# ray-project/kuberay

Hardware: NVIDIA H100
Metric: reconciles/sec over 10k RayCluster x 100 pods (batched reconcilePods + status roll-up) (higher is better)
Workload: dtype u32

## Files before the change

### kuberay_b200/csrc/kr_bucket2.cuh

```cuda
#pragma once

#include "kr_decide.cuh"

namespace kr {

__device__ __forceinline__ uint32_t inc_epoch_of(const ScratchDev &sc) { return __ldcg(&sc.inc[KR_INC_EPOCH]) + 1u; }

#ifndef KR_D2WARPS
#define KR_D2WARPS 8
#endif
static constexpr int kD2Warps = KR_D2WARPS;
#define KR_ROW_UNHEALTHY (1u << 13)
#define KR_ROW_FRESH (1u << 14)
#define KR_LG_OWNED (1u << 31)

__device__ __forceinline__ uint4 *large_slot(const ScratchDev &sc, uint32_t c, uint32_t rank) {
  if (!sc.lg) return nullptr;
  const uint4 l = __ldcg(&sc.lg[c]);
  const uint32_t j = rank - sc.bucket_stride;
  return j < l.y ? sc.region + l.x + j : nullptr;
}
__device__ __forceinline__ uint4 *rec_slot(const ScratchDev &sc, uint32_t c, uint32_t rank) {
  return rank < sc.bucket_stride ? sc.bucket + (size_t)c * sc.bucket_stride + rank : large_slot(sc, c, rank);
}
__host__ __device__ __forceinline__ uint32_t large_region_cap(uint32_t count, uint32_t stride) {
  const uint32_t want = ((count + count / 4 + 31) / 32) * 32;
  return (count > KR_LARGE_MAX_PODS ? want : (want < KR_LARGE_MAX_PODS ? want : (uint32_t)KR_LARGE_MAX_PODS)) - stride;
}


template <int kItems>
__global__ void __launch_bounds__(kSortThreads) k_match2(SnapDev s, ScratchDev sc, ResDev r, Sizes n, int has_wtd) {
  KR_TL(1);
  extern __shared__ uint32_t sm_bits[];
  __shared__ uint32_t s_orph[kSortThreads / 32];
  const uint32_t tile = blockIdx.x;
  const uint32_t warp = threadIdx.x >> 5, lane = threadIdx.x & 31;
  const uint32_t base = tile * (kSortThreads * kItems) + warp * (32 * kItems) + lane;
  uint32_t ns[kItems], cn[kItems], gn[kItems], nm[kItems], pk[kItems], ri[kItems];
#pragma unroll
  for (int it = 0; it < kItems; it++) {
    const uint32_t p = base + it * 32;
    const bool v = p < n.n_pods;
    ns[it] = v ? __ldg(&s.p_ns_id[p]) : 0u; cn[it] = v ? __ldg(&s.p_cluster_name_id[p]) : 0u;
    gn[it] = v ? __ldg(&s.p_group_name_id[p]) : 0u; nm[it] = v ? __ldg(&s.p_name_id[p]) : 0u;
    pk[it] = v ? __ldg(&s.p_packed[p]) : 0u; ri[it] = v ? (uint32_t)__ldg(&s.p_replica_index[p]) : 0u;
  }
  pdl_wait(); pdl_trigger();
  uint32_t pi[kItems];
  uint4 sl[kItems];
#pragma unroll
  for (int it = 0; it < kItems; it++) {
    pi[it] = hash_pair(ns[it], cn[it]) & sc.cl_mask;
    sl[it] = __ldg(&sc.cl_slots[pi[it]]);
  }
  if (has_wtd) {
    const uint32_t words = (sc.wt_bits_mask + 1) >> 5;
    for (uint32_t i = threadIdx.x; i < words; i += kSortThreads) sm_bits[i] = __ldcg(&sc.wt_bits[i]);
    __syncthreads();
  }
  uint32_t orphans = 0;
// ... 54 lines not shown
      const int32_t aux = aux_lookup(sc, p);
      const unsigned long long key = ((unsigned long long)p << 32) | (uint32_t)(aux + 1);
      atomicMax(reinterpret_cast<unsigned long long *>(&sc.cl_dyn[c].z), ~key);
    }
    cidx[it] = matched ? c : n.n_clusters;
    roww[it] = (slot << 16) | flags;
    orphans += __popc(__ballot_sync(0xFFFFFFFFu, v && !matched && !(pk[it] & KR_PP_TOMBSTONE)));
  }
  uint32_t rank[kItems];
#pragma unroll
  for (int it = 0; it < kItems; it++) rank[it] = cidx[it] < n.n_clusters ? atomicAdd(&sc.cl_dyn[cidx[it]].x, 1u) : 0u;
#pragma unroll
  for (int it = 0; it < kItems; it++) {
    if (cidx[it] >= n.n_clusters) continue;
    if (rank[it] < sc.bucket_stride) {
      sc.bucket[(size_t)cidx[it] * sc.bucket_stride + rank[it]] = make_uint4(base + it * 32, roww[it], ri[it], nm[it]);
      sc.pos[base + it * 32] = rank[it];
    } else if (uint4 *slot = large_slot(sc, cidx[it], rank[it])) {
      *slot = make_uint4(base + it * 32, roww[it], ri[it], nm[it]);
      sc.pos[base + it * 32] = rank[it];
    } else KR_MARK_ATTEMPT_VOID(r.totals);
  }
  if (lane == 0) s_orph[warp] = orphans;
  __syncthreads();
  if (threadIdx.x == 0) {
    uint32_t t = 0;
#pragma unroll
    for (int w = 0; w < kSortThreads / 32; w++) t += s_orph[w];
    if (t) atomicAdd(&r.totals[1], t);
  }
}


struct IncStage { uint32_t *meta; kr_cluster_result *clusters; kr_group_result *groups; uint32_t cap_clusters, cap_groups; };
// ... 156 lines not shown
    mine = c < a.r.totals[4];
    if (mine) { c = a.sc.deferred_list[c]; in_word = __ldg(&a.sc.cl_in[32 * (size_t)c + lane]); }
  } else if (kInc) {
    mine = c < __ldcg(&a.sc.inc[KR_INC_DIRTY]) && !__ldcg(&a.sc.inc[KR_INC_VOID]) && !__ldcg(&a.sc.inc[KR_INC_STRUCTURAL]);
    if (mine) {
      c = a.sc.dirty_list[c];
      in_word = __ldcg(&a.sc.cl_in[32 * (size_t)c + lane]);
    }
  }
  s_in[warp][lane] = in_word;
  __syncwarp();
  const RecordCI ci{s_in[warp]};
  if (KR_ATTEMPT_VOID(a.r.totals)) mine = false;
  if (ci.group_cnt() > KR_SMEM_GROUPS) mine = false;
  if (kInc && !mine) return;
  uint4 *bucket = a.sc.bucket + (size_t)(mine ? c : 0) * S;
  uint4 dyn = make_uint4(0, 0, 0, 0);
  uint4 recs[K] = {};
  if (mine) {
    dyn = __ldcg(&a.sc.cl_dyn[c]);
#pragma unroll
    for (int k = 0; k < K; k++) if ((uint32_t)(k * 32) + lane < S) recs[k] = __ldcg(&bucket[k * 32 + lane]);
  }
  uint32_t P = dyn.x;
  if (P > S) { mine = false; P = 0; }
  if (kInc) {
    const uint32_t epoch = inc_epoch_of(a.sc);
    const bool lost = dyn.y == epoch;
    uint32_t kept = 0, head_min = 0xFFFFFFFFu;
#pragma unroll
    for (int k = 0; k < K; k++) {
      const uint32_t j = k * 32 + lane;
      bool keep = mine && j < P;
      const bool fresh = keep && (recs[k].y & KR_ROW_FRESH);
      if (keep && lost && !fresh) keep = __ldcg(&a.sc.stamp[recs[k].x]) != epoch;
      const uint32_t bal = __ballot_sync(0xFFFFFFFFu, keep);
      if (keep) {
        uint4 rec = recs[k];
        rec.y &= ~KR_ROW_FRESH;
        const uint32_t to = kept + __popc(bal & lt);
        if (fresh || to != j) { bucket[to] = rec; if (to != j) a.sc.pos[rec.x] = to; }
        if (pp_node_type(rec.y & 0xFFFFu) == KR_NT_HEAD) head_min = min(head_min, rec.x);
      }
      kept += __popc(bal);
    }
    head_min = __reduce_min_sync(0xFFFFFFFFu, head_min);
    __syncwarp();
    unsigned long long raw = 0;
    if (mine) {
      if (lane == 0 && head_min != 0xFFFFFFFFu) raw = ~(((unsigned long long)head_min << 32) | (uint32_t)(aux_lookup(a.sc, head_min) + 1));
      raw = __shfl_sync(0xFFFFFFFFu, raw, 0);
      P = kept;
      dyn = make_uint4(kept, 0u, (uint32_t)raw, (uint32_t)(raw >> 32));
      if (lane == 0) a.sc.cl_dyn[c] = dyn;
    }
#pragma unroll
    for (int k = 0; k < K; k++) recs[k] = mine && (uint32_t)(k * 32) + lane < kept ? __ldcg(&bucket[k * 32 + lane]) : make_uint4(0, 0, 0, 0);
  }
  const uint32_t cf = ci.flags(), G = ci.group_cnt(), g0 = ci.group_off();
  const uint8_t suspend_status = ci.suspend_status(), ext_err = ci.ext_err_kind(), old_prov = ci.cond_status(KR_COND_PROVISIONED);
  const bool gate = a.f.gate_status_conditions != 0;
  if (kInc && mine) {
    uint32_t old_create = 0;
    for (uint32_t gi = lane; gi < G; gi += 32) old_create += a.r.groups[g0 + gi].n_create;
    s_old_create[warp] = __reduce_add_sync(0xFFFFFFFFu, old_create);
  }
  uint32_t head_pod = 0xFFFFFFFFu;
  int32_t head_aux = -1;
  {
    const unsigned long long raw = ((unsigned long long)dyn.w << 32) | dyn.z;
    if (mine && raw != 0) { const unsigned long long key = ~raw; head_pod = (uint32_t)(key >> 32); head_aux = (int32_t)(uint32_t)key - 1; }
  }
// ... 240 lines not shown
          __syncwarp();
#pragma unroll
          for (int k = 0; k < K; k++) {
            const bool isc = ((cand >> k) & 1u) && (pw[k] >> 16) == gi;
            if (!__any_sync(0xFFFFFFFFu, isc)) continue;
            uint32_t rank = 0;
            for (uint32_t i = 0; i < nc; i++) rank += s_list[warp][i] < pidx[k] ? 1u : 0u;
            if (isc && (int32_t)rank < pre) act[k] = KR_ACT_DELETE_RANDOM;
          }
          __syncwarp();
        }
      }
    }
  }
  if (!(cf & KR_CF_SKIP)) {
    const uint32_t head_name = (n_heads == 1 && head_pos != 0xFFFFFFFFu) ? __ldcg(&a.sc.bucket[(size_t)c * S + head_pos].w) : 0u;
    status_rollup(a.s, a.f, ci, cr, P, (uint32_t)n_heads, n_heads > 0 ? (int32_t)head_pod : -1, head_aux, head_name, ready, available, all_running);
  }
  __syncwarp();
  if (mine && lane < sizeof(kr_cluster_result) / 4)
    reinterpret_cast<uint32_t *>(&a.r.clusters[c])[lane] = reinterpret_cast<const volatile uint32_t *>(&cr)[lane];

  uint32_t n_act = 0;
  uint32_t arank[K];
#pragma unroll
  for (int k = 0; k < K; k++) {
    arank[k] = 0;
    const bool isa = act[k] != KR_ACT_KEEP;
    const uint32_t bal = __ballot_sync(0xFFFFFFFFu, isa);
    if (isa) s_list[warp][n_act + __popc(bal & lt)] = pidx[k];
    n_act += __popc(bal);
// ... 76 lines not shown
      if (want == 0) continue;
      if ((uint64_t)off + want > a.create_cap) { off += want; continue; }
      int32_t *out = a.r.create_idx + off;
      if (!a.f.gate_multihost_indexing) {
        for (uint32_t k2 = lane; k2 < want; k2 += 32) out[k2] = -1;
      } else {
        const bool mh = kMH && g_mode[gi] == GM_MULTIHOST;
        const uint64_t bound = (uint64_t)(mh ? g_mh_running[gi] : acc_list[gi] - acc_wtd[gi]) + want;
        uint32_t written = 0;
        for (uint64_t w0 = 0; w0 < bound && written < want; w0 += 1024) {
          s_bits[warp][lane] = 0;
          __syncwarp();
#pragma unroll
          for (int k = 0; k < K; k++) {
            if ((pw[k] >> 16) == gi && (pw[k] & KR_PP_HAS_REPLICA_IDX) && (mh ? ((mh_head >> k) & 1u) != 0 : (act[k] == KR_ACT_KEEP && pidx[k] != 0xFFFFFFFFu))) {
              const int32_t idx = (int32_t)__ldcg(&a.sc.bucket[(size_t)c * S + k * 32 + lane].z);
              if (idx >= 0 && (uint64_t)idx >= w0 && (uint64_t)idx < w0 + 1024 && (uint64_t)idx < bound)
                atomicOr(&s_bits[warp][(idx - w0) >> 5], 1u << ((idx - w0) & 31));
            }
          }
          __syncwarp();
          const uint32_t word = s_bits[warp][lane];
          const uint64_t wbase = w0 + 32ull * lane;
          uint32_t freeb = ~word;
          if (wbase >= bound) freeb = 0;
          else if (bound - wbase < 32) freeb &= (1u << (uint32_t)(bound - wbase)) - 1;
          const uint32_t cnt = __popc(freeb);
          uint32_t x = cnt;
#pragma unroll
          for (int d = 1; d < 32; d <<= 1) { const uint32_t y = __shfl_up_sync(0xFFFFFFFFu, x, d); if (lane >= (uint32_t)d) x += y; }
          uint32_t pos = written + x - cnt;
// ... 22 lines not shown
```

### kuberay_b200/csrc/kr_common.cuh

```cuda
#pragma once

#include <cuda_runtime.h>
#include <stdint.h>

#include "../../include/kr_engine.h"

namespace kr {


struct SnapDev {
  const uint32_t *c_ns_id, *c_name_id;
  const uint64_t *c_uid_hash;
  const uint32_t *c_flags;
  const uint8_t *c_suspend_status, *c_ext_err_kind;
  const uint32_t *c_ext_err_msg_id, *c_group_off, *c_group_cnt;
  const uint64_t *c_json_off;
  const uint32_t *c_json_len;
  const uint8_t *c_old_state;
  const int32_t *c_old_counts;
  const uint8_t *c_old_cond_status, *c_old_cond_variant;
  const uint32_t *c_old_cond_reason_id, *c_old_cond_msg_id, *c_old_head_ids;
  const uint8_t *c_svc_count, *c_svc_ip_kind;
  const uint32_t *c_svc_ip_id, *c_svc_name_id;
  const uint32_t *g_cluster_idx, *g_name_id;
// ... 34 lines not shown
  uint32_t *aux_keys; uint32_t *aux_vals; uint32_t aux_mask;
  uint4 *rows;
  uint32_t *keys[2]; uint32_t *vals[2];
  uint32_t *hist;
  uint32_t *row_total;
  uint32_t *gcreate;
  uint32_t *cact;
  uint32_t *mh_rep, *mh_name, *mh_meta, *mh_cnt, *mh_flg;
  uint8_t *mh_act, *mh_head;
  uint32_t *act_tmp_idx; uint8_t *act_tmp_code;
  uint32_t *tile_orph;
  uint32_t *chain;
  uint32_t *ccount, *cstart;
  uint32_t *deferred_list;
  int32_t *gacc;
  uint4 *bucket; uint32_t bucket_stride;
  uint32_t *wt_bits; uint32_t wt_bits_mask;
  uint32_t *cl_in;
  uint4 *cl_dyn;
  uint32_t *stamp;
  uint32_t *touched;
  uint32_t *touched_old;
  uint32_t *pos;
  uint32_t *dirty_flag;
  uint32_t *obj_flag;
  uint32_t *dirty_list;
  uint32_t *act_res, *cre_res;
  uint32_t *inc;
  uint4 *lg;
  uint4 *region;
};
enum {
  KR_INC_TOUCHED = 0, KR_INC_DIRTY = 1,
  KR_INC_STRUCTURAL = 2,
  KR_INC_EPOCH = 3,
  KR_INC_HEADS = 4,
  KR_INC_VOID = 5,
  KR_INC_GROUPS = 6,
  KR_INC_LSEG = 7,
  KR_INC_GROW = 8,
  KR_INC_SPILL = 9,
  KR_INC_GROWN = 10,
};
enum {
  KR_CI_FLAGS = 0, KR_CI_GOFF = 1, KR_CI_GCNT = 2,
// ... 100 lines not shown
```

### kuberay_b200/csrc/kr_engine.cu

```cuda
#include <cuda_runtime.h>

#include <algorithm>
#include <chrono>
#include <cstdarg>
#include <cstdio>
#include <cstdlib>
#include <cstring>
#include <string>
#include <thread>
#include <unordered_map>
#include <unordered_set>
#include <vector>

#include "kr_kernels.cuh"
#include "kr_incr.cuh"
#include "kr_large.cuh"
#include "kr_huge.cuh"

using namespace kr;

int kr_specjson_emit_string(const uint8_t *spec_json, uint64_t len, bool muted, long max_groups, std::string &out, long *n_groups);

namespace {

// ... 389 lines not shown
  L.cstart = o; o = align_up(o + 4 * ((size_t)n.n_clusters + 2));
  L.tile_orph = o; o = align_up(o + 4 * ((size_t)L.mtiles + 8));
  L.mh_rep = o; o = align_up(o + 4 * (size_t)n.n_pods);
  L.mh_name = o; o = align_up(o + 4 * (size_t)n.n_pods);
  L.mh_meta = o; o = align_up(o + 4 * (size_t)n.n_pods);
  L.mh_cnt = o; o = align_up(o + 4 * (size_t)n.n_pods);
  L.mh_flg = o; o = align_up(o + 4 * (size_t)n.n_pods);
  L.mh_act = o; o = align_up(o + (size_t)n.n_pods);
  L.mh_head = o; o = align_up(o + (size_t)n.n_pods);
  L.act_tmp_idx = o; o = align_up(o + 4 * (size_t)n.n_pods);
  L.act_tmp_code = o; o = align_up(o + (size_t)n.n_pods);
  L.bucket_entries = std::max<size_t>(4 * (size_t)n.n_pods, 64 * (size_t)n.n_clusters);
  L.bucket_entries = std::max<size_t>(L.bucket_entries, std::min<size_t>(256 * (size_t)n.n_clusters, (size_t)4 << 20));
  if (64 * (size_t)n.n_clusters > 8 * (size_t)n.n_pods + (4u << 20)) L.bucket_entries = 0;
  L.cl_in = o; o = align_up(o + 128 * (size_t)n.n_clusters);
  L.bucket = o; o = align_up(o + 16 * L.bucket_entries);
  L.inc_zero = o;
  L.stamp = o; o = align_up(o + 4 * (size_t)n.n_pods);
  L.dirty_flag = o; o = align_up(o + 4 * (size_t)n.n_clusters);
  L.obj_flag = o; o = align_up(o + 4 * (size_t)n.n_clusters);
  L.inc = o; o = align_up(o + 64);
  L.inc_zero_end = o;
  L.touched = o; o = align_up(o + 4 * (size_t)n.n_pods);
  L.touched_old = o; o = align_up(o + 4 * (size_t)n.n_pods);
  L.pos = o; o = align_up(o + 4 * (size_t)n.n_pods);
  L.dirty_list = o; o = align_up(o + 4 * (size_t)n.n_clusters);
  L.act_res = o; o = align_up(o + 4 * (size_t)n.n_clusters);
  L.cre_res = o; o = align_up(o + 4 * (size_t)n.n_clusters);
  L.total = o;
  return L;
}
// ... 64 lines not shown
  bool env_radix = false;
  uint32_t *h_totals = nullptr;
  bool no_bucket = false;
  bool hash_spin = true;
  uint32_t bstride = 0;
  bool large_on = false;
  bool wide_on = false;
  bool huge_on = false;
  std::vector<uint32_t> large_rows; std::vector<uint2> large_reg;
  bool lg_stale = false;
  bool lg_moved = false;
  uint32_t n_large = 0;
  uint32_t n_lsort = 0;
  uint32_t n_tiles = 0;
  uint8_t *d_lg = nullptr;
  uint4 *d_region = nullptr;
  size_t large_entries = 0;
  std::vector<uint4> h_lg; std::vector<uint32_t> h_lg_list;
  uint8_t *d_huge = nullptr;
  size_t huge_tiles = 0;
  std::vector<uint4> h_tiles;
  bool huge_growth = false;
  size_t huge_reserve = 0;
  bool large_growth = false;
  uint4 *d_grow = nullptr; uint4 *h_grow = nullptr;
  size_t lg_cursor = 0;
  bool ran_bucket = false;
  uint64_t h2d_accum = 0;
  uint32_t *h_order = nullptr, *d_order = nullptr;
  cudaEvent_t ev_order = nullptr;
  bool order_pending = false;
// ... 95 lines not shown
  s.vals[0] = reinterpret_cast<uint32_t *>(b + L.vals0); s.vals[1] = reinterpret_cast<uint32_t *>(b + L.vals1);
  s.hist = reinterpret_cast<uint32_t *>(b + L.hist);
  s.row_total = reinterpret_cast<uint32_t *>(b + L.row_total);
  s.gacc = reinterpret_cast<int32_t *>(b + L.gacc);
  s.gcreate = reinterpret_cast<uint32_t *>(b + L.gcreate);
  s.deferred_list = reinterpret_cast<uint32_t *>(b + L.deferred_list);
  s.cact = reinterpret_cast<uint32_t *>(b + L.cact);
  s.ccount = reinterpret_cast<uint32_t *>(b + L.ccount);
  s.chain = reinterpret_cast<uint32_t *>(b + L.chain);
  s.cstart = reinterpret_cast<uint32_t *>(b + L.cstart);
  s.tile_orph = reinterpret_cast<uint32_t *>(b + L.tile_orph);
  s.mh_rep = reinterpret_cast<uint32_t *>(b + L.mh_rep); s.mh_name = reinterpret_cast<uint32_t *>(b + L.mh_name);
  s.mh_meta = reinterpret_cast<uint32_t *>(b + L.mh_meta); s.mh_cnt = reinterpret_cast<uint32_t *>(b + L.mh_cnt);
  s.mh_flg = reinterpret_cast<uint32_t *>(b + L.mh_flg); s.mh_act = b + L.mh_act; s.mh_head = b + L.mh_head;
  s.act_tmp_idx = reinterpret_cast<uint32_t *>(b + L.act_tmp_idx); s.act_tmp_code = b + L.act_tmp_code;
  s.bucket = reinterpret_cast<uint4 *>(b + L.bucket); s.bucket_stride = 0;
  s.wt_bits = reinterpret_cast<uint32_t *>(b + L.wt_bits); s.wt_bits_mask = L.wt_bits_n - 1;
  s.cl_in = reinterpret_cast<uint32_t *>(b + L.cl_in);
  s.cl_dyn = reinterpret_cast<uint4 *>(b + L.cl_dyn);
  s.stamp = reinterpret_cast<uint32_t *>(b + L.stamp); s.touched = reinterpret_cast<uint32_t *>(b + L.touched);
  s.touched_old = reinterpret_cast<uint32_t *>(b + L.touched_old); s.pos = reinterpret_cast<uint32_t *>(b + L.pos);
  s.obj_flag = reinterpret_cast<uint32_t *>(b + L.obj_flag);
  s.dirty_flag = reinterpret_cast<uint32_t *>(b + L.dirty_flag); s.dirty_list = reinterpret_cast<uint32_t *>(b + L.dirty_list);
  s.act_res = reinterpret_cast<uint32_t *>(b + L.act_res); s.cre_res = reinterpret_cast<uint32_t *>(b + L.cre_res);
  s.inc = reinterpret_cast<uint32_t *>(b + L.inc);
  s.lg = nullptr; s.region = nullptr;
  return s;
}

template <typename... KArgs, typename... Args>
cudaError_t launch_pdl(void (*kern)(KArgs...), dim3 grid, dim3 block, size_t smem, cudaStream_t st, bool pdl, Args... args) {
// ... 1033 lines not shown
    e->lg_stale = true;
    return KR_OK;
  }
  if (option == KR_OPT_LARGE_CLUSTERS || option == KR_OPT_WIDE_CLUSTERS || option == KR_OPT_HUGE_CLUSTERS) {
    bool &on = option == KR_OPT_LARGE_CLUSTERS ? e->large_on : option == KR_OPT_WIDE_CLUSTERS ? e->wide_on : e->huge_on;
    if (on == (value != 0)) return KR_OK;
    if (value) CK(cudaSetDevice(e->cfg.device));
    if (value && option != KR_OPT_HUGE_CLUSTERS && !e->d_lg) {
      const size_t Nc = e->cfg.max_clusters;
      CK(cudaMalloc((void **)&e->d_lg, align_up(16 * Nc) + 4 * Nc));
      CK(cudaMemset(e->d_lg, 0, align_up(16 * Nc)));
    }
    if (value && option == KR_OPT_LARGE_CLUSTERS && !e->d_region) {
      const size_t Np = e->cfg.max_pods;
      const size_t entries = Np * 5 / 4 + 32 * (Np / 257 + 1);
      CK(cudaMalloc((void **)&e->d_region, 16 * entries));
      e->large_entries = entries;
    }
    if (value && option == KR_OPT_HUGE_CLUSTERS && !e->d_huge) {
      e->huge_tiles = resident_tiles(e->cfg);
      if (int rc = alloc_huge(e, 0)) return rc;
    }
    on = value != 0;
    if (int rc = drop_regions(e, 0)) return rc;
    e->lg_cursor = 0; e->lg_stale = true; e->inc_valid = false; e->gvalid = false;
    e->force_radix = e->env_radix;
    if (e->begun) e->bstride = first_stride(e->sizes);
    return KR_OK;
  }
  if (option == KR_OPT_BUCKET_STRIDE) return fail(e, KR_E_INVALID, "KR_OPT_BUCKET_STRIDE can only be read");
  return fail(e, KR_E_INVALID, "unknown option %u", option);
// ... 645 lines not shown
```

### kuberay_b200/csrc/kr_huge.cuh

```cuda
#pragma once

#include "kr_large.cuh"

namespace kr {

static constexpr int kHugeThreads = 1024;
static constexpr int kHugePer = kHugeTile / kHugeThreads;

struct HugeDev {
  const uint4 *tiles;
  uint32_t *cnt;
  uint32_t *done;
  uint32_t *runs;
  uint32_t *stash;
};

__device__ __forceinline__ uint32_t gallop_lower_bound(const uint32_t *s, uint32_t lo, uint32_t n, uint32_t x) {
  uint32_t hi = lo, step = 1;
  while (hi < n && s[hi] < x) { lo = hi + 1; hi += step; step <<= 1; }
  hi = min(hi, n);
  while (lo < hi) { const uint32_t mid = (lo + hi) >> 1; if (s[mid] < x) lo = mid + 1; else hi = mid; }
  return lo;
}

// ... 15 lines not shown
    const uint32_t cap = __ldcg(&sc.lg[c].y);
    bool go = !KR_ATTEMPT_VOID(a.r.totals);
    if (kInc) go = go && !__ldcg(&sc.inc[KR_INC_VOID]) && !__ldcg(&sc.inc[KR_INC_STRUCTURAL]) && __ldcg(&sc.dirty_flag[c]) == epoch;
    const bool wide = a.s.c_group_cnt[c] > KR_SMEM_GROUPS;
    s_go = go && (P > S ? P - S <= cap : wide);
    if (!s_go && r0 == 0) sc.lg[c].w = 0;
  }
  __syncthreads();
  if (!s_go) return;
  const bool lost = kInc && dyn.y == epoch;
  const uint32_t r1 = min(P, r0 + (uint32_t)kHugeTile), n = r1 > r0 ? r1 - r0 : 0u;
  const uint32_t per = (n + kHugeThreads - 1) / kHugeThreads;
  const uint32_t j0 = r0 + min(tid * per, n), j1 = min(j0 + per, r1);
  uint32_t kept = 0;
  for (uint32_t j = j0; j < j1; j++) {
    const uint4 rec = __ldcg(rec_slot(sc, c, j));
    const bool keep = !lost || (rec.y & KR_ROW_FRESH) || __ldcg(&sc.stamp[rec.x]) != epoch;
    if (keep) { sc.rows[rec.x] = make_uint4(rec.w, a.s.p_replica_name_id[rec.x], rec.z, rec.y & ~KR_ROW_FRESH); kept++; }
  }
  uint32_t x = kept;
#pragma unroll
  for (int d = 1; d < 32; d <<= 1) { const uint32_t y = __shfl_up_sync(0xFFFFFFFFu, x, d); if (lane >= (uint32_t)d) x += y; }
  if (lane == 31) s_warp[warp] = x;
  __syncthreads();
  uint32_t before = 0, total = 0;
  for (uint32_t w = 0; w < kHugeThreads / 32; w++) { const uint32_t v = s_warp[w]; before += w < warp ? v : 0u; total += v; }
  uint32_t o = before + x - kept;
  uint32_t *stash = h.stash + (size_t)blockIdx.x * kHugeTile;
  for (uint32_t j = j0; j < j1; j++) {
    const uint4 rec = __ldcg(rec_slot(sc, c, j));
    const bool keep = !lost || (rec.y & KR_ROW_FRESH) || __ldcg(&sc.stamp[rec.x]) != epoch;
    if (keep) { s_idx[o] = rec.x; stash[o] = rec.x; o++; }
  }
  block_sort_asc<kHugeThreads>(s_idx, total, tid);
  uint32_t *run = h.runs + (size_t)blockIdx.x * kHugeTile;
  for (uint32_t k = tid; k < total; k += kHugeThreads) run[k] = s_idx[k];
  if (tid == 0) {
    h.cnt[blockIdx.x] = total;
    __threadfence();
    if (atomicAdd(&h.done[t.z], 1u) == t.w - 1) {
      __threadfence();
      uint32_t sum = 0;
      for (uint32_t i = t.z; i < t.z + t.w; i++) sum += __ldcg(&h.cnt[i]);
      const uint32_t seg = atomicAdd(&sc.inc[KR_INC_LSEG], sum);
      sc.lg[c].z = seg; sc.lg[c].w = sum | KR_LG_OWNED;
// ... 34 lines not shown
    const uint32_t *run = h.runs + (size_t)u * kHugeTile;
    for (uint32_t k = tid; k < n_u; k += kHugeThreads) s_run[k] = __ldcg(run + k);
    __syncthreads();
    if (k0 >= n_me) continue;
    uint32_t lo = 0;
#pragma unroll
    for (int i = 0; i < kHugePer; i++) { lo = gallop_lower_bound(s_run, lo, n_u, v[i]); at[i] += lo; }
  }
#pragma unroll
  for (int i = 0; i < kHugePer; i++) if (k0 + i < n_me) a.r.sorted_pod_idx[seg + at[i]] = v[i];
  if (kInc) {
    const uint32_t *stash = h.stash + (size_t)me * kHugeTile;
    for (uint32_t k = tid; k < n_me; k += kHugeThreads) {
      const uint32_t p = __ldcg(stash + k);
      const uint4 row = __ldcg(&sc.rows[p]);
      *rec_slot(sc, c, base + k) = make_uint4(p, row.w, row.z, row.x);
      sc.pos[p] = base + k;
    }
    if (me == t.z && tid == 0) { sc.cl_dyn[c].x = total; sc.cl_dyn[c].y = 0u; }
  }
}

}
```

### kuberay_b200/csrc/kr_incr.cuh

```cuda
#pragma once

#include "kr_bucket2.cuh"

namespace kr {

__device__ __forceinline__ uint32_t inc_epoch(const ScratchDev &sc) { return inc_epoch_of(sc); }

__device__ __forceinline__ void mark_dirty(const ScratchDev &sc, uint32_t c, uint32_t epoch) {
  if (atomicExch(&sc.dirty_flag[c], epoch) != epoch) sc.dirty_list[atomicAdd(&sc.inc[KR_INC_DIRTY], 1u)] = c;
}

__device__ __forceinline__ bool cl_probe(const ScratchDev &sc, uint32_t ns, uint32_t name, uint32_t &c, uint32_t &cflags, uint32_t &gname0) {
  if (name == 0) return false;
  uint32_t i = hash_pair(ns, name) & sc.cl_mask;
  while (true) {
    const uint4 q = __ldcg(&sc.cl_slots[i]);
    if (q.x == name && q.y == ns) { c = q.w >> 2; cflags = q.w & 3u; gname0 = q.z; return true; }
    if (q.x == KR_EMPTY32 && q.y == KR_EMPTY32) return false;
    i = (i + 1) & sc.cl_mask;
  }
}

__device__ __forceinline__ bool inc_touch(const SnapDev &s, const ScratchDev &sc, const ResDev &r, uint32_t p, uint32_t epoch, uint32_t n_resident, uint32_t &ns, uint32_t &nm) {
  if (atomicExch(&sc.stamp[p], epoch) == epoch) return false;
// ... 213 lines not shown

__global__ void __launch_bounds__(256) k_inc_refresh(SnapDev s, ScratchDev sc) {
  const uint32_t n_dirty = __ldcg(&sc.inc[KR_INC_DIRTY]);
  const uint32_t epoch = inc_epoch(sc);
  if (__ldcg(&sc.inc[KR_INC_STRUCTURAL])) return;
  for (uint32_t i = blockIdx.x * blockDim.x + threadIdx.x; i < n_dirty; i += gridDim.x * blockDim.x) {
    const uint32_t c = sc.dirty_list[i];
    if (__ldcg(&sc.obj_flag[c]) == epoch) write_cl_in(s, sc, c, s.c_group_off[c], s.c_group_cnt[c]);
  }
}

static constexpr uint32_t kGrowResult = KR_GROW_MAX, kGrowSpill = 2 * KR_GROW_MAX;
static constexpr size_t kGrowBytes = 16 * ((size_t)kGrowSpill + 2 * (size_t)KR_GROW_SPILL);

__device__ __noinline__ bool grow_spill(const uint4 *lg, uint32_t *inc, uint32_t *pos, uint32_t stride, uint4 *grow, uint32_t c,
                                        uint32_t rank, uint4 rec) {
  const uint4 l = __ldcg(&lg[c]);
  if (rank == stride + l.y) {
    const uint32_t j = atomicAdd(&inc[KR_INC_GROW], 1u);
    if (j >= KR_GROW_MAX) return false;
    grow[j] = make_uint4(c, l.x, l.y, 0u);
  }
  const uint32_t k = atomicAdd(&inc[KR_INC_SPILL], 1u);
  if (k >= KR_GROW_SPILL) return false;
  grow[kGrowSpill + 2 * k] = make_uint4(rec.x, rank, c, 0u);
  grow[kGrowSpill + 2 * k + 1] = rec;
  pos[rec.x] = rank;
  return true;
}

__global__ void __launch_bounds__(256) k_inc_admit(SnapDev s, ScratchDev sc, ResDev r, Sizes n, int has_wtd, uint4 *grow) {
  const uint32_t n_touched = __ldcg(&sc.inc[KR_INC_TOUCHED]);
  const uint32_t epoch = inc_epoch(sc);
  if (__ldcg(&sc.inc[KR_INC_STRUCTURAL])) return;
  for (uint32_t i = blockIdx.x * blockDim.x + threadIdx.x; i < n_touched; i += gridDim.x * blockDim.x) {
    const uint32_t p = sc.touched[i], c_old = sc.touched_old[i];
    if (p >= n.n_pods) continue;
    const uint32_t ns = s.p_ns_id[p], cn = s.p_cluster_name_id[p], gn = s.p_group_name_id[p], nm = s.p_name_id[p], pk = s.p_packed[p];
    const uint32_t ri = (uint32_t)s.p_replica_index[p];
    uint32_t c = n.n_clusters, cflags = 0, gname0 = 0;
    const bool matched = cl_probe(sc, ns, cn, c, cflags, gname0);
    uint32_t slot = KR_ROW_NO_GROUP, g0 = 0xFFFFFFFFu;
    if (matched && gn != 0) {
      if (gname0 == gn) slot = 0;
      else if (cflags & KR_CL_MULTI) {
        const uint4 rec = sc.cl_rec[c];
        g0 = rec.x;
        for (uint32_t gi = 1; gi < rec.y; gi++)
          if (s.g_name_id[g0 + gi] == gn) { slot = gi; break; }
      }
    }
    uint32_t flags = pk & (0x7FFu | KR_PP_TOMBSTONE);
    if (should_delete(pk)) flags |= KR_ROW_UNHEALTHY;
    if (has_wtd) {
// ... 8 lines not shown
              atomicMin(&r.wtd_pod_idx[e], p);
              if (slot != KR_ROW_NO_GROUP) {
                if (g0 == 0xFFFFFFFFu) g0 = s.c_group_off[c];
                const uint32_t g = g0 + slot, off = s.g_wtd_off[g];
                if (e >= off && e < off + s.g_wtd_cnt[g]) flags |= KR_ROW_WTD_OWN;
              }
            }
            break;
          }
          j = (j + 1) & sc.wt_mask;
          kk = __ldcg(&sc.wt_keys[j]);
        }
      }
    }
    if (matched && c == c_old) {
      uint4 *at = rec_slot(sc, c, sc.pos[p]);
      if (!at) { sc.inc[KR_INC_VOID] = 1u; continue; }
      *at = make_uint4(p, (slot << 16) | flags, ri, nm);
      sc.stamp[p] = 0u;
      continue;
    }
    if (c_old != KR_EMPTY32) sc.cl_dyn[c_old].y = epoch;
    if (!matched) {
      if (!(pk & KR_PP_TOMBSTONE)) atomicAdd(&r.totals[1], 1u);
      continue;
    }
    mark_dirty(sc, c, epoch);
    const uint32_t rank = atomicAdd(&sc.cl_dyn[c].x, 1u);
    const uint4 rec = make_uint4(p, (slot << 16) | flags | KR_ROW_FRESH, ri, nm);
    if (uint4 *at = rec_slot(sc, c, rank)) { *at = rec; sc.pos[p] = rank; }
    else if (!grow || !grow_spill(sc.lg, sc.inc, sc.pos, sc.bucket_stride, grow, c, rank, rec)) sc.inc[KR_INC_VOID] = 1u;
  }
}

__global__ void __launch_bounds__(256) k_inc_clusters_insert(SnapDev s, ScratchDev sc, ResDev r, const uint32_t *rows, uint32_t n, int names) {
  const uint32_t i = blockIdx.x * blockDim.x + threadIdx.x;
  if (i >= n || __ldcg(&sc.inc[KR_INC_STRUCTURAL])) return;
  const uint32_t c = rows[i];
  cl_insert_cluster(s, sc, c);
  sc.cl_dyn[c] = make_uint4(0u, 0u, 0u, 0u);
  sc.act_res[c] = 0u; sc.cre_res[c] = 0u;
  r.act_start[c] = 0u; r.act_cnt[c] = 0u;
  if (sc.lg) sc.lg[c] = make_uint4(0u, 0u, 0u, 0u);
  const uint32_t g0 = s.c_group_off[c], G = s.c_group_cnt[c];
  for (uint32_t g = g0; g < g0 + G; g++) {
// ... 44 lines not shown

__global__ void __launch_bounds__(256) k_inc_digest_move(const uint32_t *__restrict__ pairs, uint32_t n, char *hash) {
  const uint32_t t = blockIdx.x * blockDim.x + threadIdx.x;
  if (t >= 2 * n) return;
  const uint32_t from = pairs[2 * (t >> 1)], to = pairs[2 * (t >> 1) + 1];
  reinterpret_cast<uint4 *>(hash + 32 * (size_t)to)[t & 1] = reinterpret_cast<const uint4 *>(hash + 32 * (size_t)from)[t & 1];
}

__global__ void __launch_bounds__(256) k_inc_clusters_release(SnapDev s, ScratchDev sc, ResDev r, const uint32_t *gone, uint32_t n_gone, uint32_t n_resident) {
  const uint32_t w = (blockIdx.x * blockDim.x + threadIdx.x) >> 5, lane = threadIdx.x & 31;
  if (w >= n_gone) return;
  const uint32_t o = gone[w], epoch = inc_epoch(sc);
  const uint4 rec = sc.cl_rec[o];
  const uint32_t P = sc.cl_dyn[o].x;
  for (uint32_t k = lane; k < P; k += 32) {
    const uint4 *at = rec_slot(sc, o, k);
    uint32_t ns, nm;
    if (at) inc_touch(s, sc, r, at->x, epoch, n_resident, ns, nm);
  }
  uint32_t cre = 0;
  for (uint32_t g = rec.x + lane; g < rec.x + rec.y; g += 32) cre += r.groups[g].n_create;
  cre = __reduce_add_sync(0xFFFFFFFFu, cre);
  if (lane == 0) {
    if (r.act_cnt[o]) atomicSub(&r.totals[2], r.act_cnt[o]);
    if (cre) atomicSub(&r.totals[6], cre);
  }
}

__global__ void __launch_bounds__(256) k_inc_large_release(SnapDev s, ScratchDev sc, ResDev r, const uint4 *gone, uint32_t n_resident) {
  __shared__ uint32_t s_cre[8];
  const uint4 g = gone[blockIdx.x];
  const uint32_t o = g.x, S = sc.bucket_stride, epoch = inc_epoch(sc), tid = threadIdx.x;
  const uint32_t P = min(__ldcg(&sc.cl_dyn[o].x), S + g.z);
  for (uint32_t k = tid; k < P; k += blockDim.x) {
    const uint4 *at = k < S ? sc.bucket + (size_t)o * S + k : sc.region + g.y + (k - S);
    uint32_t ns, nm;
    inc_touch(s, sc, r, at->x, epoch, n_resident, ns, nm);
  }
  const uint4 rec = sc.cl_rec[o];
  uint32_t cre = 0;
  for (uint32_t gi = rec.x + tid; gi < rec.x + rec.y; gi += blockDim.x) cre += r.groups[gi].n_create;
  cre = __reduce_add_sync(0xFFFFFFFFu, cre);
  if ((tid & 31) == 0) s_cre[tid >> 5] = cre;
  __syncthreads();
  if (tid == 0) {
    cre = 0;
    for (uint32_t w = 0; w < blockDim.x / 32; w++) cre += s_cre[w];
    if (r.act_cnt[o]) atomicSub(&r.totals[2], r.act_cnt[o]);
    if (cre) atomicSub(&r.totals[6], cre);
  }
// ... 59 lines not shown
```

### kuberay_b200/csrc/kr_large.cuh

```cuda
#pragma once

#include "kr_incr.cuh"

namespace kr {

static constexpr int kLargeSortThreads = 512;
static constexpr int kLargeDecideThreads = 128;
static constexpr int kHugeDecideThreads = 512;
static constexpr int kHugeTile = KR_LARGE_MAX_PODS;

template <int kThreads>
__device__ __forceinline__ void block_sort_asc(uint32_t *s, uint32_t total, uint32_t tid) {
  uint32_t n2 = 2;
  while (n2 < total) n2 <<= 1;
  for (uint32_t k = total + tid; k < n2; k += kThreads) s[k] = 0xFFFFFFFFu;
  __syncthreads();
  for (uint32_t size = 2; size <= n2; size <<= 1) {
    for (uint32_t stride = size >> 1; stride > 0; stride >>= 1) {
      for (uint32_t t = tid; t < n2 / 2; t += kThreads) {
        const uint32_t lo = 2 * stride * (t / stride) + (t % stride), hi = lo + stride;
        const bool asc = (lo & size) == 0;
        const uint32_t u = s[lo], v = s[hi];
        if ((u > v) == asc) { s[lo] = v; s[hi] = u; }
      }
// ... 42 lines not shown
    return;
  }
  for (uint32_t i = blockIdx.x; i < n; i += gridDim.x)
    if (!kHuge || s_e[i].z <= KR_LARGE_MAX_PODS)
      for (uint32_t j = tid; j < s_e[i].z; j += blockDim.x) sc.region[s_off[i] + j] = __ldcg(&sc.region[s_e[i].y + j]);
  if (kHuge)
    for (uint32_t i = 0; i < n; i++)
      if (s_e[i].z > KR_LARGE_MAX_PODS)
        for (uint32_t j = blockIdx.x * blockDim.x + tid; j < s_e[i].z; j += gridDim.x * blockDim.x) sc.region[s_off[i] + j] = __ldcg(&sc.region[s_e[i].y + j]);
  const uint32_t n_spill = __ldcg(&sc.inc[KR_INC_SPILL]);
  for (uint32_t k = blockIdx.x * blockDim.x + tid; k < n_spill && k < KR_GROW_SPILL; k += gridDim.x * blockDim.x) {
    const uint4 at = __ldcg(&grow[kGrowSpill + 2 * k]);
    uint32_t lo = 0, hi = n - 1;
    while (lo < hi) { const uint32_t mid = (lo + hi) >> 1; if (s_e[mid].x < at.z) lo = mid + 1; else hi = mid; }
    if (s_e[lo].x != at.z || at.y < S + s_e[lo].z || at.y - S >= s_cap[lo]) { sc.inc[KR_INC_VOID] = 1u; continue; }
    sc.region[s_off[lo] + at.y - S] = __ldcg(&grow[kGrowSpill + 2 * k + 1]);
  }
  if (blockIdx.x == 0) {
    if (tid < n) {
      sc.lg[s_e[tid].x] = make_uint4(s_off[tid], s_cap[tid], 0u, 0u);
      grow[kGrowResult + tid] = make_uint4(s_e[tid].x, s_off[tid], s_cap[tid], s_new[tid]);
    }
    if (tid == 0) sc.inc[KR_INC_GROWN] = n;
    if (kHuge) {
      for (uint32_t t = tid; t < n_tiles; t += blockDim.x) {
        const uint32_t c = tiles[t].x;
        uint32_t lo = 0, hi = n - 1;
        while (lo < hi) { const uint32_t mid = (lo + hi) >> 1; if (s_e[mid].x < c) lo = mid + 1; else hi = mid; }
        if (s_e[lo].x == c) tiles[t].x = KR_EMPTY32;
      }
      if (tid == 0) {
// ... 34 lines not shown
  if (tid == 0) {
    const uint32_t cap = __ldcg(&sc.lg[c].y);
    sc.lg[c].w = 0;
    bool go = !KR_ATTEMPT_VOID(a.r.totals);
    if (kInc) go = go && !__ldcg(&sc.inc[KR_INC_VOID]) && !__ldcg(&sc.inc[KR_INC_STRUCTURAL]) && __ldcg(&sc.dirty_flag[c]) == epoch;
    const bool wide = a.s.c_group_cnt[c] > KR_SMEM_GROUPS;
    s_seg = go && (P > S ? P - S <= cap : wide) && S + cap <= KR_LARGE_MAX_PODS;
  }
  __syncthreads();
  if (!s_seg) return;
  const bool lost = kInc && dyn.y == epoch;
  const uint32_t per = (P + kLargeSortThreads - 1) / kLargeSortThreads;
  const uint32_t j0 = min(tid * per, P), j1 = min(j0 + per, P);
  uint32_t kept = 0;
  for (uint32_t j = j0; j < j1; j++) {
    const uint4 rec = __ldcg(rec_slot(sc, c, j));
    const bool keep = !lost || (rec.y & KR_ROW_FRESH) || __ldcg(&sc.stamp[rec.x]) != epoch;
    if (keep) { sc.rows[rec.x] = make_uint4(rec.w, a.s.p_replica_name_id[rec.x], rec.z, rec.y & ~KR_ROW_FRESH); kept++; }
  }
  uint32_t x = kept;
#pragma unroll
  for (int d = 1; d < 32; d <<= 1) { const uint32_t y = __shfl_up_sync(0xFFFFFFFFu, x, d); if (lane >= (uint32_t)d) x += y; }
  if (lane == 31) s_warp[warp] = x;
  __syncthreads();
  uint32_t before = 0, total = 0;
  for (uint32_t w = 0; w < kLargeSortThreads / 32; w++) { const uint32_t v = s_warp[w]; before += w < warp ? v : 0u; total += v; }
  uint32_t o = before + x - kept;
  for (uint32_t j = j0; j < j1; j++) {
    const uint4 rec = __ldcg(rec_slot(sc, c, j));
    const bool keep = !lost || (rec.y & KR_ROW_FRESH) || __ldcg(&sc.stamp[rec.x]) != epoch;
    if (keep) s_idx[o++] = rec.x;
  }
  if (tid == 0) {
    s_seg = atomicAdd(&sc.inc[KR_INC_LSEG], total);
    if ((uint64_t)s_seg + total > a.n.n_pods) {
      if (kInc) sc.inc[KR_INC_VOID] = 1u; else KR_MARK_ATTEMPT_VOID(a.r.totals);
    }
  }
  __syncthreads();
  const uint32_t seg = s_seg;
  if ((uint64_t)seg + total > a.n.n_pods) return;
  if (kInc) {
    for (uint32_t k = tid; k < total; k += kLargeSortThreads) {
      const uint32_t p = s_idx[k];
      const uint4 row = sc.rows[p];
      *rec_slot(sc, c, k) = make_uint4(p, row.w, row.z, row.x);
      sc.pos[p] = k;
    }
    if (tid == 0) { sc.cl_dyn[c].x = total; sc.cl_dyn[c].y = 0u; }
  }
  block_sort_asc<kLargeSortThreads>(s_idx, total, tid);
  for (uint32_t k = tid; k < total; k += kLargeSortThreads) a.r.sorted_pod_idx[seg + k] = s_idx[k];
  if (tid == 0) { sc.lg[c].z = seg; sc.lg[c].w = total | KR_LG_OWNED; }
}

template <bool kInc, int kThreads>
__global__ void __launch_bounds__(kThreads, 1) k_decide_large(Decide2Args a, const uint32_t *__restrict__ lg_list, uint32_t n_list, uint32_t n_lsort,
                                                           const uint4 *grown) {
  constexpr int kWarps = kThreads / 32;
  constexpr bool kHugePart = kThreads != kLargeDecideThreads;
  __shared__ int32_t s_acc[4][KR_SMEM_GROUPS];
// ... 88 lines not shown
```

Baseline: 82.49 million.

## Shrink per-pod bucket records from uint4 to uint2 and reload fields on demand

Bucket and large-region records now hold only the pod index and the row word, cut from 16 bytes to 8. Name and replica index are no longer copied into the records. They are read from the snapshot arrays at the few places that need them: head name, replica bits, and rows rebuild in the large and huge paths. This halves bucket write and read traffic in match and decide, at the cost of extra gathered loads in those rarer paths.

```diff
diff --git a/kuberay_b200/csrc/kr_bucket2.cuh b/kuberay_b200/csrc/kr_bucket2.cuh
--- a/kuberay_b200/csrc/kr_bucket2.cuh
+++ b/kuberay_b200/csrc/kr_bucket2.cuh
@@ -14,13 +14,13 @@
 #define KR_ROW_FRESH (1u << 14)
 #define KR_LG_OWNED (1u << 31)
 
-__device__ __forceinline__ uint4 *large_slot(const ScratchDev &sc, uint32_t c, uint32_t rank) {
+__device__ __forceinline__ uint2 *large_slot(const ScratchDev &sc, uint32_t c, uint32_t rank) {
   if (!sc.lg) return nullptr;
   const uint4 l = __ldcg(&sc.lg[c]);
   const uint32_t j = rank - sc.bucket_stride;
   return j < l.y ? sc.region + l.x + j : nullptr;
 }
-__device__ __forceinline__ uint4 *rec_slot(const ScratchDev &sc, uint32_t c, uint32_t rank) {
+__device__ __forceinline__ uint2 *rec_slot(const ScratchDev &sc, uint32_t c, uint32_t rank) {
   return rank < sc.bucket_stride ? sc.bucket + (size_t)c * sc.bucket_stride + rank : large_slot(sc, c, rank);
 }
 __host__ __device__ __forceinline__ uint32_t large_region_cap(uint32_t count, uint32_t stride) {
@@ -37,14 +37,14 @@
   const uint32_t tile = blockIdx.x;
   const uint32_t warp = threadIdx.x >> 5, lane = threadIdx.x & 31;
   const uint32_t base = tile * (kSortThreads * kItems) + warp * (32 * kItems) + lane;
-  uint32_t ns[kItems], cn[kItems], gn[kItems], nm[kItems], pk[kItems], ri[kItems];
+  uint32_t ns[kItems], cn[kItems], gn[kItems], nm[kItems], pk[kItems];
 #pragma unroll
   for (int it = 0; it < kItems; it++) {
     const uint32_t p = base + it * 32;
     const bool v = p < n.n_pods;
     ns[it] = v ? __ldg(&s.p_ns_id[p]) : 0u; cn[it] = v ? __ldg(&s.p_cluster_name_id[p]) : 0u;
     gn[it] = v ? __ldg(&s.p_group_name_id[p]) : 0u; nm[it] = v ? __ldg(&s.p_name_id[p]) : 0u;
-    pk[it] = v ? __ldg(&s.p_packed[p]) : 0u; ri[it] = v ? (uint32_t)__ldg(&s.p_replica_index[p]) : 0u;
+    pk[it] = v ? __ldg(&s.p_packed[p]) : 0u;
   }
   pdl_wait(); pdl_trigger();
   uint32_t pi[kItems];
@@ -129,10 +129,10 @@
   for (int it = 0; it < kItems; it++) {
     if (cidx[it] >= n.n_clusters) continue;
     if (rank[it] < sc.bucket_stride) {
-      sc.bucket[(size_t)cidx[it] * sc.bucket_stride + rank[it]] = make_uint4(base + it * 32, roww[it], ri[it], nm[it]);
+      sc.bucket[(size_t)cidx[it] * sc.bucket_stride + rank[it]] = make_uint2(base + it * 32, roww[it]);
       sc.pos[base + it * 32] = rank[it];
-    } else if (uint4 *slot = large_slot(sc, cidx[it], rank[it])) {
-      *slot = make_uint4(base + it * 32, roww[it], ri[it], nm[it]);
+    } else if (uint2 *slot = large_slot(sc, cidx[it], rank[it])) {
+      *slot = make_uint2(base + it * 32, roww[it]);
       sc.pos[base + it * 32] = rank[it];
     } else KR_MARK_ATTEMPT_VOID(r.totals);
   }
@@ -319,9 +319,9 @@
   if (KR_ATTEMPT_VOID(a.r.totals)) mine = false;
   if (ci.group_cnt() > KR_SMEM_GROUPS) mine = false;
   if (kInc && !mine) return;
-  uint4 *bucket = a.sc.bucket + (size_t)(mine ? c : 0) * S;
+  uint2 *bucket = a.sc.bucket + (size_t)(mine ? c : 0) * S;
   uint4 dyn = make_uint4(0, 0, 0, 0);
-  uint4 recs[K] = {};
+  uint2 recs[K] = {};
   if (mine) {
     dyn = __ldcg(&a.sc.cl_dyn[c]);
 #pragma unroll
@@ -341,7 +341,7 @@
       if (keep && lost && !fresh) keep = __ldcg(&a.sc.stamp[recs[k].x]) != epoch;
       const uint32_t bal = __ballot_sync(0xFFFFFFFFu, keep);
       if (keep) {
-        uint4 rec = recs[k];
+        uint2 rec = recs[k];
         rec.y &= ~KR_ROW_FRESH;
         const uint32_t to = kept + __popc(bal & lt);
         if (fresh || to != j) { bucket[to] = rec; if (to != j) a.sc.pos[rec.x] = to; }
@@ -360,7 +360,7 @@
       if (lane == 0) a.sc.cl_dyn[c] = dyn;
     }
 #pragma unroll
-    for (int k = 0; k < K; k++) recs[k] = mine && (uint32_t)(k * 32) + lane < kept ? __ldcg(&bucket[k * 32 + lane]) : make_uint4(0, 0, 0, 0);
+    for (int k = 0; k < K; k++) recs[k] = mine && (uint32_t)(k * 32) + lane < kept ? __ldcg(&bucket[k * 32 + lane]) : make_uint2(0, 0);
   }
   const uint32_t cf = ci.flags(), G = ci.group_cnt(), g0 = ci.group_off();
   const uint8_t suspend_status = ci.suspend_status(), ext_err = ci.ext_err_kind(), old_prov = ci.cond_status(KR_COND_PROVISIONED);
@@ -631,7 +631,7 @@
     }
   }
   if (!(cf & KR_CF_SKIP)) {
-    const uint32_t head_name = (n_heads == 1 && head_pos != 0xFFFFFFFFu) ? __ldcg(&a.sc.bucket[(size_t)c * S + head_pos].w) : 0u;
+    const uint32_t head_name = (n_heads == 1 && head_pos != 0xFFFFFFFFu) ? __ldg(&s.p_name_id[head_pod]) : 0u;
     status_rollup(a.s, a.f, ci, cr, P, (uint32_t)n_heads, n_heads > 0 ? (int32_t)head_pod : -1, head_aux, head_name, ready, available, all_running);
   }
   __syncwarp();
@@ -738,7 +738,7 @@
 #pragma unroll
           for (int k = 0; k < K; k++) {
             if ((pw[k] >> 16) == gi && (pw[k] & KR_PP_HAS_REPLICA_IDX) && (mh ? ((mh_head >> k) & 1u) != 0 : (act[k] == KR_ACT_KEEP && pidx[k] != 0xFFFFFFFFu))) {
-              const int32_t idx = (int32_t)__ldcg(&a.sc.bucket[(size_t)c * S + k * 32 + lane].z);
+              const int32_t idx = __ldg(&s.p_replica_index[pidx[k]]);
               if (idx >= 0 && (uint64_t)idx >= w0 && (uint64_t)idx < w0 + 1024 && (uint64_t)idx < bound)
                 atomicOr(&s_bits[warp][(idx - w0) >> 5], 1u << ((idx - w0) & 31));
             }
diff --git a/kuberay_b200/csrc/kr_common.cuh b/kuberay_b200/csrc/kr_common.cuh
--- a/kuberay_b200/csrc/kr_common.cuh
+++ b/kuberay_b200/csrc/kr_common.cuh
@@ -72,7 +72,7 @@
   uint32_t *ccount, *cstart;
   uint32_t *deferred_list;
   int32_t *gacc;
-  uint4 *bucket; uint32_t bucket_stride;
+  uint2 *bucket; uint32_t bucket_stride;
   uint32_t *wt_bits; uint32_t wt_bits_mask;
   uint32_t *cl_in;
   uint4 *cl_dyn;
@@ -86,7 +86,7 @@
   uint32_t *act_res, *cre_res;
   uint32_t *inc;
   uint4 *lg;
-  uint4 *region;
+  uint2 *region;
 };
 enum {
   KR_INC_TOUCHED = 0, KR_INC_DIRTY = 1,
diff --git a/kuberay_b200/csrc/kr_engine.cu b/kuberay_b200/csrc/kr_engine.cu
--- a/kuberay_b200/csrc/kr_engine.cu
+++ b/kuberay_b200/csrc/kr_engine.cu
@@ -427,7 +427,7 @@
   L.bucket_entries = std::max<size_t>(L.bucket_entries, std::min<size_t>(256 * (size_t)n.n_clusters, (size_t)4 << 20));
   if (64 * (size_t)n.n_clusters > 8 * (size_t)n.n_pods + (4u << 20)) L.bucket_entries = 0;
   L.cl_in = o; o = align_up(o + 128 * (size_t)n.n_clusters);
-  L.bucket = o; o = align_up(o + 16 * L.bucket_entries);
+  L.bucket = o; o = align_up(o + sizeof(uint2) * L.bucket_entries);
   L.inc_zero = o;
   L.stamp = o; o = align_up(o + 4 * (size_t)n.n_pods);
   L.dirty_flag = o; o = align_up(o + 4 * (size_t)n.n_clusters);
@@ -522,7 +522,7 @@
   uint32_t n_lsort = 0;
   uint32_t n_tiles = 0;
   uint8_t *d_lg = nullptr;
-  uint4 *d_region = nullptr;
+  uint2 *d_region = nullptr;
   size_t large_entries = 0;
   std::vector<uint4> h_lg; std::vector<uint32_t> h_lg_list;
   uint8_t *d_huge = nullptr;
@@ -648,7 +648,7 @@
   s.mh_meta = reinterpret_cast<uint32_t *>(b + L.mh_meta); s.mh_cnt = reinterpret_cast<uint32_t *>(b + L.mh_cnt);
   s.mh_flg = reinterpret_cast<uint32_t *>(b + L.mh_flg); s.mh_act = b + L.mh_act; s.mh_head = b + L.mh_head;
   s.act_tmp_idx = reinterpret_cast<uint32_t *>(b + L.act_tmp_idx); s.act_tmp_code = b + L.act_tmp_code;
-  s.bucket = reinterpret_cast<uint4 *>(b + L.bucket); s.bucket_stride = 0;
+  s.bucket = reinterpret_cast<uint2 *>(b + L.bucket); s.bucket_stride = 0;
   s.wt_bits = reinterpret_cast<uint32_t *>(b + L.wt_bits); s.wt_bits_mask = L.wt_bits_n - 1;
   s.cl_in = reinterpret_cast<uint32_t *>(b + L.cl_in);
   s.cl_dyn = reinterpret_cast<uint4 *>(b + L.cl_dyn);
@@ -1712,7 +1712,7 @@
     if (value && option == KR_OPT_LARGE_CLUSTERS && !e->d_region) {
       const size_t Np = e->cfg.max_pods;
       const size_t entries = Np * 5 / 4 + 32 * (Np / 257 + 1);
-      CK(cudaMalloc((void **)&e->d_region, 16 * entries));
+      CK(cudaMalloc((void **)&e->d_region, sizeof(uint2) * entries));
       e->large_entries = entries;
     }
     if (value && option == KR_OPT_HUGE_CLUSTERS && !e->d_huge) {
diff --git a/kuberay_b200/csrc/kr_huge.cuh b/kuberay_b200/csrc/kr_huge.cuh
--- a/kuberay_b200/csrc/kr_huge.cuh
+++ b/kuberay_b200/csrc/kr_huge.cuh
@@ -53,9 +53,12 @@
   const uint32_t j0 = r0 + min(tid * per, n), j1 = min(j0 + per, r1);
   uint32_t kept = 0;
   for (uint32_t j = j0; j < j1; j++) {
-    const uint4 rec = __ldcg(rec_slot(sc, c, j));
+    const uint2 rec = __ldcg(rec_slot(sc, c, j));
     const bool keep = !lost || (rec.y & KR_ROW_FRESH) || __ldcg(&sc.stamp[rec.x]) != epoch;
-    if (keep) { sc.rows[rec.x] = make_uint4(rec.w, a.s.p_replica_name_id[rec.x], rec.z, rec.y & ~KR_ROW_FRESH); kept++; }
+    if (keep) {
+      sc.rows[rec.x] = make_uint4(a.s.p_name_id[rec.x], a.s.p_replica_name_id[rec.x], (uint32_t)a.s.p_replica_index[rec.x], rec.y & ~KR_ROW_FRESH);
+      kept++;
+    }
   }
   uint32_t x = kept;
 #pragma unroll
@@ -67,7 +70,7 @@
   uint32_t o = before + x - kept;
   uint32_t *stash = h.stash + (size_t)blockIdx.x * kHugeTile;
   for (uint32_t j = j0; j < j1; j++) {
-    const uint4 rec = __ldcg(rec_slot(sc, c, j));
+    const uint2 rec = __ldcg(rec_slot(sc, c, j));
     const bool keep = !lost || (rec.y & KR_ROW_FRESH) || __ldcg(&sc.stamp[rec.x]) != epoch;
     if (keep) { s_idx[o] = rec.x; stash[o] = rec.x; o++; }
   }
@@ -132,7 +135,7 @@
     for (uint32_t k = tid; k < n_me; k += kHugeThreads) {
       const uint32_t p = __ldcg(stash + k);
       const uint4 row = __ldcg(&sc.rows[p]);
-      *rec_slot(sc, c, base + k) = make_uint4(p, row.w, row.z, row.x);
+      *rec_slot(sc, c, base + k) = make_uint2(p, row.w);
       sc.pos[p] = base + k;
     }
     if (me == t.z && tid == 0) { sc.cl_dyn[c].x = total; sc.cl_dyn[c].y = 0u; }
diff --git a/kuberay_b200/csrc/kr_incr.cuh b/kuberay_b200/csrc/kr_incr.cuh
--- a/kuberay_b200/csrc/kr_incr.cuh
+++ b/kuberay_b200/csrc/kr_incr.cuh
@@ -251,7 +251,7 @@
 static constexpr size_t kGrowBytes = 16 * ((size_t)kGrowSpill + 2 * (size_t)KR_GROW_SPILL);
 
 __device__ __noinline__ bool grow_spill(const uint4 *lg, uint32_t *inc, uint32_t *pos, uint32_t stride, uint4 *grow, uint32_t c,
-                                        uint32_t rank, uint4 rec) {
+                                        uint32_t rank, uint2 rec) {
   const uint4 l = __ldcg(&lg[c]);
   if (rank == stride + l.y) {
     const uint32_t j = atomicAdd(&inc[KR_INC_GROW], 1u);
@@ -261,7 +261,7 @@
   const uint32_t k = atomicAdd(&inc[KR_INC_SPILL], 1u);
   if (k >= KR_GROW_SPILL) return false;
   grow[kGrowSpill + 2 * k] = make_uint4(rec.x, rank, c, 0u);
-  grow[kGrowSpill + 2 * k + 1] = rec;
+  grow[kGrowSpill + 2 * k + 1] = make_uint4(rec.x, rec.y, 0u, 0u);
   pos[rec.x] = rank;
   return true;
 }
@@ -274,7 +274,6 @@
     const uint32_t p = sc.touched[i], c_old = sc.touched_old[i];
     if (p >= n.n_pods) continue;
     const uint32_t ns = s.p_ns_id[p], cn = s.p_cluster_name_id[p], gn = s.p_group_name_id[p], nm = s.p_name_id[p], pk = s.p_packed[p];
-    const uint32_t ri = (uint32_t)s.p_replica_index[p];
     uint32_t c = n.n_clusters, cflags = 0, gname0 = 0;
     const bool matched = cl_probe(sc, ns, cn, c, cflags, gname0);
     uint32_t slot = KR_ROW_NO_GROUP, g0 = 0xFFFFFFFFu;
@@ -313,9 +312,9 @@
       }
     }
     if (matched && c == c_old) {
-      uint4 *at = rec_slot(sc, c, sc.pos[p]);
+      uint2 *at = rec_slot(sc, c, sc.pos[p]);
       if (!at) { sc.inc[KR_INC_VOID] = 1u; continue; }
-      *at = make_uint4(p, (slot << 16) | flags, ri, nm);
+      *at = make_uint2(p, (slot << 16) | flags);
       sc.stamp[p] = 0u;
       continue;
     }
@@ -326,8 +325,8 @@
     }
     mark_dirty(sc, c, epoch);
     const uint32_t rank = atomicAdd(&sc.cl_dyn[c].x, 1u);
-    const uint4 rec = make_uint4(p, (slot << 16) | flags | KR_ROW_FRESH, ri, nm);
-    if (uint4 *at = rec_slot(sc, c, rank)) { *at = rec; sc.pos[p] = rank; }
+    const uint2 rec = make_uint2(p, (slot << 16) | flags | KR_ROW_FRESH);
+    if (uint2 *at = rec_slot(sc, c, rank)) { *at = rec; sc.pos[p] = rank; }
     else if (!grow || !grow_spill(sc.lg, sc.inc, sc.pos, sc.bucket_stride, grow, c, rank, rec)) sc.inc[KR_INC_VOID] = 1u;
   }
 }
@@ -402,7 +401,7 @@
   const uint4 rec = sc.cl_rec[o];
   const uint32_t P = sc.cl_dyn[o].x;
   for (uint32_t k = lane; k < P; k += 32) {
-    const uint4 *at = rec_slot(sc, o, k);
+    const uint2 *at = rec_slot(sc, o, k);
     uint32_t ns, nm;
     if (at) inc_touch(s, sc, r, at->x, epoch, n_resident, ns, nm);
   }
@@ -421,7 +420,7 @@
   const uint32_t o = g.x, S = sc.bucket_stride, epoch = inc_epoch(sc), tid = threadIdx.x;
   const uint32_t P = min(__ldcg(&sc.cl_dyn[o].x), S + g.z);
   for (uint32_t k = tid; k < P; k += blockDim.x) {
-    const uint4 *at = k < S ? sc.bucket + (size_t)o * S + k : sc.region + g.y + (k - S);
+    const uint2 *at = k < S ? sc.bucket + (size_t)o * S + k : sc.region + g.y + (k - S);
     uint32_t ns, nm;
     inc_touch(s, sc, r, at->x, epoch, n_resident, ns, nm);
   }
diff --git a/kuberay_b200/csrc/kr_large.cuh b/kuberay_b200/csrc/kr_large.cuh
--- a/kuberay_b200/csrc/kr_large.cuh
+++ b/kuberay_b200/csrc/kr_large.cuh
@@ -80,7 +80,8 @@
     uint32_t lo = 0, hi = n - 1;
     while (lo < hi) { const uint32_t mid = (lo + hi) >> 1; if (s_e[mid].x < at.z) lo = mid + 1; else hi = mid; }
     if (s_e[lo].x != at.z || at.y < S + s_e[lo].z || at.y - S >= s_cap[lo]) { sc.inc[KR_INC_VOID] = 1u; continue; }
-    sc.region[s_off[lo] + at.y - S] = __ldcg(&grow[kGrowSpill + 2 * k + 1]);
+    const uint4 rec = __ldcg(&grow[kGrowSpill + 2 * k + 1]);
+    sc.region[s_off[lo] + at.y - S] = make_uint2(rec.x, rec.y);
   }
   if (blockIdx.x == 0) {
     if (tid < n) {
@@ -145,9 +146,12 @@
   const uint32_t j0 = min(tid * per, P), j1 = min(j0 + per, P);
   uint32_t kept = 0;
   for (uint32_t j = j0; j < j1; j++) {
-    const uint4 rec = __ldcg(rec_slot(sc, c, j));
+    const uint2 rec = __ldcg(rec_slot(sc, c, j));
     const bool keep = !lost || (rec.y & KR_ROW_FRESH) || __ldcg(&sc.stamp[rec.x]) != epoch;
-    if (keep) { sc.rows[rec.x] = make_uint4(rec.w, a.s.p_replica_name_id[rec.x], rec.z, rec.y & ~KR_ROW_FRESH); kept++; }
+    if (keep) {
+      sc.rows[rec.x] = make_uint4(a.s.p_name_id[rec.x], a.s.p_replica_name_id[rec.x], (uint32_t)a.s.p_replica_index[rec.x], rec.y & ~KR_ROW_FRESH);
+      kept++;
+    }
   }
   uint32_t x = kept;
 #pragma unroll
@@ -158,7 +162,7 @@
   for (uint32_t w = 0; w < kLargeSortThreads / 32; w++) { const uint32_t v = s_warp[w]; before += w < warp ? v : 0u; total += v; }
   uint32_t o = before + x - kept;
   for (uint32_t j = j0; j < j1; j++) {
-    const uint4 rec = __ldcg(rec_slot(sc, c, j));
+    const uint2 rec = __ldcg(rec_slot(sc, c, j));
     const bool keep = !lost || (rec.y & KR_ROW_FRESH) || __ldcg(&sc.stamp[rec.x]) != epoch;
     if (keep) s_idx[o++] = rec.x;
   }
@@ -175,7 +179,7 @@
     for (uint32_t k = tid; k < total; k += kLargeSortThreads) {
       const uint32_t p = s_idx[k];
       const uint4 row = sc.rows[p];
-      *rec_slot(sc, c, k) = make_uint4(p, row.w, row.z, row.x);
+      *rec_slot(sc, c, k) = make_uint2(p, row.w);
       sc.pos[p] = k;
     }
     if (tid == 0) { sc.cl_dyn[c].x = total; sc.cl_dyn[c].y = 0u; }
```

After: 85.44 million (median of 6 runs). 1.04x the previous value.
